# adam-ikari/uvhttp

Measured on AMD Instinct MI355X. Metric: WebSocket payload unmask GiB/s (device-resident), 64 KiB frames, 1/2/4/8 GPU, higher is better.
Workload: dtype u8; 1 GPU; C3: 65536 x 64 KiB masked BINARY frames per GPU (C5 shard shape); mode=inplace, frames_per_gpu=65536, payload_bytes_per_frame=65536, wire_bytes_per_frame=65550, parallelism=shard1 (independent frames, no collective)

## Files before the change

uvhttp_amd/__init__.py:

```python
from __future__ import annotations

import ctypes as C
import os

__all__ = [
    "lib", "LIB_PATH", "FrameHeader", "FrameDesc", "MessageDesc", "BatchSummary", "Batch",
    "WsConnectionStruct", "parse_frame_header", "apply_mask", "WsConnection", "GpuEngine",
    "GpuError", "OPCODES", "FRAME_STATUS", "gen_frame_stride", "GpuPipeline", "Stream",
    "StreamResult", "STREAM_DT", "STREAM_RESULT_DT", "STREAM_RESULT_BYTES", "Batcher",
]

_HERE = os.path.dirname(os.path.abspath(__file__))
LIB_PATH = os.path.join(_HERE, "lib", "libuvhttp_ws_amd.so")
TESTHOOKS_LIB_PATH = os.path.join(_HERE, "lib", "libuvhttp_ws_amd_testhooks.so")

OPCODES = dict(CONTINUATION=0x0, TEXT=0x1, BINARY=0x2, CLOSE=0x8, PING=0x9, PONG=0xA)
FRAME_STATUS = {
    0: "OK", 1: "INCOMPLETE", 2: "SKIPPED", -1: "ERR_PARSE", -2: "ERR_RSV", -3: "ERR_CONTROL",
    -4: "ERR_UNMASKED", -5: "ERR_TOO_BIG", -6: "ERR_BUFFER", -7: "ERR_FRAGMENT",
    -8: "ERR_MESSAGE", -9: "ERR_LAYOUT", -10: "ERR_CAPACITY", -11: "ERR_DEVICE",
}
FLAG_FIN, FLAG_MASK, FLAG_MSG_END = 0x01, 0x02, 0x20


# ... 201 lines not shown
    if _LIB is None:
        _LIB = load_library(LIB_PATH)
    return _LIB


_TESTHOOKS = None


def test_hooks_library() -> C.CDLL:
    global _TESTHOOKS
    if _TESTHOOKS is None:
        _TESTHOOKS = load_library(TESTHOOKS_LIB_PATH)
    return _TESTHOOKS


EXPERIMENT_KNOBS = (
    "UVHTTP_WS_MAX_POLLS", "UVHTTP_WS_SCRATCH_POOL", "UVHTTP_WS_PLAN_FPT", "UVHTTP_WS_EPOCH_START",
    "UVHTTP_WS_BUILD_SMALL", "UVHTTP_WS_FUSED", "UVHTTP_WS_FUSED_MAX", "UVHTTP_WS_PLAN_WIDE",
    "UVHTTP_WS_REC_SCAN", "UVHTTP_WS_BUILD_FRAMES", "UVHTTP_WS_COMPACT", "UVHTTP_WS_WALK_SINGLE",
    "UVHTTP_WS_WALK_FUSE", "UVHTTP_WS_DESC_SCAN", "UVHTTP_WS_WALK_REC",
    "UVHTTP_WS_WALK", "UVHTTP_WS_TIME_CHAIN", "UVHTTP_WS_SPEC", "UVHTTP_WS_SPEC_MAX",
    "UVHTTP_WS_SUMMARY_FAST", "UVHTTP_WS_TILE", "UVHTTP_WS_TIMING_FENCE", "UVHTTP_WS_PIPE_IN_FLIGHT",
    "UVHTTP_TLS_CRYPT_GRID", "UVHTTP_WS_BATCHER_TRACE", "UVHTTP_WS_BATCHER_FAIL_EVERY",
    "UVHTTP_WS_COPY_SSE2", "UVHTTP_WS_DESC_EMIT", "UVHTTP_WS_STREAM_SPEC")


def experiment_knobs_set():
    return [k for k in EXPERIMENT_KNOBS if k in os.environ]


def default_library() -> C.CDLL:
    return test_hooks_library() if experiment_knobs_set() else lib()


def load_library(path: str) -> C.CDLL:
    if not os.path.exists(path):
        raise ImportError(f"{path} missing: run `make` (or __graft_entry__.build())")
    try:
        import torch
    except ImportError:
        pass
    L = C.CDLL(path)
    vp, u32, u64, i32 = C.c_void_p, C.c_uint32, C.c_uint64, C.c_int32
    sig = {
        "uvhttp_ws_amd_version": (C.c_char_p, []),
        "uvhttp_ws_parse_frame_header": (C.c_int, [vp, C.c_size_t, C.POINTER(FrameHeader),
                                                   C.POINTER(C.c_size_t)]),
# ... 881 lines not shown
```

uvhttp_amd/csrc/ws_gpu.hip:

```cpp
#include <hip/hip_runtime.h>

#include <stdint.h>
#include <stdio.h>
#include <stdlib.h>
#include <string.h>

#include <vector>

#include "uvhttp_ws_amd.h"
#include "ws_engine_int.h"

namespace {

constexpr int kBlock = 256;
constexpr uint64_t kMapTile = 16384;
constexpr uint64_t kScatterAvg = 26624;
constexpr uint32_t kMaxFrames = 1u << 26;
constexpr uint32_t kNoFrame = 0xFFFFFFFFu;
constexpr uint32_t kMaxEpoch = (1u << 30) - 1;

typedef uint32_t u32x4 __attribute__((ext_vector_type(4)));

struct ScanElem {
    int32_t last_data;
// ... 157 lines not shown
    ScanElem* group_agg;
    ScanElem* block_incl;
    ScanElem* block_excl;
    LbRec* rec_a;
    LbRec* rec_p;
    uint32_t* counters;
    uint64_t* tile_first;
    uint64_t* first_bad;
    uint64_t* spec_bad;
    uint64_t* arena_first;
    uint32_t* ctl;
    void* recs;
    void* parts;
    uint8_t* info;
};

constexpr int kCtlEpoch = 0;
constexpr int kCtlDone = 1;
constexpr int kCtlFaultEp = 2;
constexpr int kCtlFaults = 3;
constexpr int kCtlGate = 4;
constexpr int kCtlSpecOff = 5;
constexpr int kCtlSpecBreak = 6;
constexpr int kCtlWords = 7;
constexpr uint32_t kMaxHostEpoch = kMaxEpoch / 2;

__device__ inline uint64_t tag_of(uint32_t epoch, uint32_t frame) {
    return ((uint64_t)epoch << 32) | (uint32_t)~frame;
}
__device__ inline void tag_claim(uint64_t* p, uint32_t epoch, uint32_t frame, uint32_t cas) {
    unsigned long long* q = reinterpret_cast<unsigned long long*>(p);
    const unsigned long long mine = tag_of(epoch, frame);
    if (!cas) {
        atomicMax(q, mine);
        return;
    }
    unsigned long long cur = atomicMax(q, mine);
    while ((uint32_t)(cur >> 32) > epoch) {
        const unsigned long long seen = atomicCAS(q, cur, mine);
        if (seen == cur) return;
        cur = seen;
        if ((uint32_t)(cur >> 32) <= epoch) {
            atomicMax(q, mine);
            return;
        }
    }
}
// ... 105 lines not shown
    uint64_t frame_stride;
    double stride_inv;
    FrameRec8* recs;
    uint32_t n;
    int32_t max_frame_size;
    int32_t max_message_size;
    int32_t is_server;
    uint64_t n_tiles;
    uint8_t* arena;
    uint64_t arena_cap;
    uint64_t n_arena_tiles;
    const uvhttp_ws_stream_t* streams;
    const uint32_t* n_dev;
    uvhttp_ws_stream_result_t* s_results;
    const uint32_t* s_over;
    uint32_t n_streams;
    uint32_t epoch;
    uint32_t dev_epoch;
    uint32_t max_polls;
    uvhttp_ws_batch_summary_t* summary;
    uint32_t plan_frames;
    uint64_t* stamp;
    uint64_t spec_P;
    uint32_t gate;
    uint32_t cas_claims;
    uvhttp_ws_message_desc_t* msgs;
};

constexpr uint32_t kStampRing = 128, kStampKinds = 16, kStampBegin = 256, kStampEnd = 4096;
constexpr uint64_t kStampPer = kStampBegin + kStampEnd;
constexpr uint64_t kStampLow = (1ull << 40) - 1;
constexpr uint32_t kStampTagPeriod = (1u << 24) - 1;
constexpr uint64_t kStampWords = (uint64_t)kStampRing * kStampKinds * kStampPer;

__host__ __device__ inline uint32_t stamp_tag(uint32_t epoch) { return epoch % kStampTagPeriod + 1u; }
__device__ inline uint64_t* stamp_slot(uint64_t* st, uint32_t epoch, uint32_t kind) {
    return st + ((uint64_t)(epoch % kStampRing) * kStampKinds + kind) * kStampPer;
}
__host__ __device__ inline bool stamp_sampled(uint64_t g) {
    return g < 1024 || (g < 65536 ? (g & 63) == 63 : (g & 1023) == 1023);
}
__host__ __device__ inline uint32_t stamp_end_word(uint64_t g, uint32_t wave) {
    const uint64_t blk = g < 1024 ? g : g < 65536 ? 1024 + (g >> 6) : 2048 + (g >> 10);
    return (uint32_t)((blk * 4 + (wave & 3)) % kStampEnd);
}
__device__ inline uint64_t stamp_clock() {
// ... 497 lines not shown
template <int FPT>
__device__ inline void plan_pass2(const BatchArgs& a, uvhttp_ws_frame_desc_t* desc,
                                  uvhttp_ws_message_desc_t* msgs, const Workspace& ws, uint32_t i0,
                                  uint32_t n, ScanElem run, uvhttp_ws_frame_desc_t (&dv)[FPT]) {
#pragma unroll
    for (int k = 0; k < FPT; ++k) {
        const uint32_t i = i0 + k;
        if (i < n) {
            const SegInfo g = seg_info(a, i, n);
            ScanElem e = scan_identity();
            if (dv[k].status == UVHTTP_WS_FRAME_OK) e = scan_elem_of(dv[k], (int32_t)i, g.head);
            else if (g.head) e.bits = kHead;
            resolve_one(a, msgs, ws, i, n, g, run, dv[k]);
            store_desc(desc, i, dv[k]);
            run = scan_combine(run, e);
        }
    }
}

template <int FPT, int NT = kBlock, bool REC = false>
__global__ __launch_bounds__(NT) void k_plan(BatchArgs a, uvhttp_ws_frame_desc_t* desc,
                                                 uvhttp_ws_message_desc_t* msgs, Workspace ws) {
    resolve_epoch(a, ws);
    if (a.gate && ws.ctl[kCtlGate] != a.epoch) return;
    StampScope stamp_(a.stamp, a.epoch, UVHTTP_WS_STAMP_PLAN);
    __shared__ uint32_t s_ticket;
    if (threadIdx.x == 0) {
        const uint32_t t =
            __hip_atomic_fetch_add(&ws.counters[0], 1u, __ATOMIC_RELAXED, __HIP_MEMORY_SCOPE_AGENT);
        if (t + 1 == gridDim.x)
            __hip_atomic_store(&ws.counters[0], 0u, __ATOMIC_RELAXED, __HIP_MEMORY_SCOPE_AGENT);
        s_ticket = t;
    }
    __syncthreads();
    const uint32_t b = s_ticket;
    const uint32_t n = nframes(a);
    const uint32_t i0 = (b * NT + threadIdx.x) * FPT;
    if constexpr (REC) {
        ScanElem tagg = scan_identity();
        FrameRec8 r[FPT];
        const uint32_t ilast = n ? n - 1 : 0;
#pragma unroll
        for (int k = 0; k < FPT; ++k) r[k] = a.recs[i0 + k < n ? i0 + k : ilast];
#pragma unroll
        for (int k = 0; k < FPT; ++k) {
            const uint32_t i = i0 + k;
            if (i < n) {
// ... 225 lines not shown
    if (pe <= va || ps >= va + 16) return;
    const uint32_t rk = rotr32(key, 8u * (uint32_t)((va - ps) & 3u));
    if (ps <= va && va + 16 <= pe) {
        m = u32x4{rk, rk, rk, rk};
        return;
    }
    const int lo = ps > va ? (int)(ps - va) : 0;
    const int hi = pe < va + 16 ? (int)(pe - va) : 16;
    m.x |= rk & lane_bytes(lo, hi, 0);
    m.y |= rk & lane_bytes(lo, hi, 1);
    m.z |= rk & lane_bytes(lo, hi, 2);
    m.w |= rk & lane_bytes(lo, hi, 3);
}

__device__ inline bool any_bits(const u32x4& m) { return (m.x | m.y | m.z | m.w) != 0u; }

constexpr int kStoreAux = 18;
__host__ inline void inplace_tile_shape(uint64_t avg, int& blk, int& vpt) {
    if (avg >= 12288) blk = 64, vpt = 1;
    else if (avg >= 2560) blk = 64, vpt = 2;
    else blk = 256, vpt = avg >= 2048 ? 2 : 4;
}

constexpr uint32_t kFastFrames = 8;
template <int BLOCK, int VPT>
__device__ __forceinline__ void unmask_tile(BatchArgs a,
                                            const uvhttp_ws_frame_desc_t* __restrict__ desc,
                                            const Workspace& ws, uint64_t tile_base,
                                            uint32_t& n_out, uint32_t& nb_out, StampScope& ss) {
    constexpr uint64_t kT = (uint64_t)BLOCK * VPT * 16;
    __shared__ uint64_t s_ps[BLOCK];
    __shared__ uint64_t s_pe[BLOCK];
    __shared__ uint32_t s_key[BLOCK];

    const uint64_t t0 = (tile_base + ss.anchor_s(blockIdx.x)) * kT;
    const uint64_t vend = a.wire_len;
    const uint64_t full_end = vend & ~(uint64_t)15;
    const uint64_t clamp_va = full_end ? full_end - 16 : 0;

    u32x4 data[VPT];
    uint64_t va[VPT];
#pragma unroll
    for (int v = 0; v < VPT; ++v) {
        va[v] = t0 + ((uint64_t)v * BLOCK + threadIdx.x) * 16u;
        const uint64_t la = va[v] < full_end ? va[v] : clamp_va;
        data[v] = __builtin_nontemporal_load(reinterpret_cast<const u32x4*>(a.wire + la));
    }

    resolve_epoch(a, ws);
    const uint32_t n = nframes(a);
    const uint32_t nb = first_bad_of(a, ws, n);
    n_out = n;
    nb_out = nb;
    if (nb == 0 || n == 0 || t0 >= vend) return;
    const uint32_t last = (nb < n ? nb : n) - 1;
    const uint64_t c0 = t0 / kMapTile, c1 = (t0 + kT - 1) / kMapTile + 1;
    const uint32_t f0 = tag_get(ws.tile_first[c0], a.epoch, kNoFrame);
    uint32_t f1 = (c1 < a.n_tiles) ? tag_get(ws.tile_first[c1], a.epoch, kNoFrame) : last;
    if (f0 > last) return;
    if (f1 > last || f1 < f0) f1 = last;

    u32x4 m[VPT];
#pragma unroll
    for (int v = 0; v < VPT; ++v) m[v] = u32x4{0, 0, 0, 0};

    if (f1 - f0 < kFastFrames) {
        if (a.streams) {
            for (uint32_t f = f0; f <= f1; ++f) {
                const uint64_t ps = desc[f].payload_off;
                const uint64_t len = desc[f].payload_len;
                const uint32_t key = desc[f].masking_key;
// ... 67 lines not shown
                const uint32_t mw[4] = {m[v].x, m[v].y, m[v].z, m[v].w};
                for (uint64_t bq = 0; full_end + bq < vend; ++bq) {
                    const uint8_t mb = (uint8_t)(mw[bq >> 2] >> (8 * (bq & 3)));
                    if (mb) a.wire[full_end + bq] ^= mb;
                }
            }
        }
    }
}

__device__ inline void device_result(uvhttp_ws_stream_result_t& r);
__device__ inline void capacity_result(uvhttp_ws_stream_result_t& r);
__device__ inline void stream_fix(const BatchArgs& a, const Workspace& ws) {
    const bool fault = ws.ctl[kCtlFaultEp] == a.epoch;
    if (!fault && *a.s_over != a.epoch) return;
    for (uint32_t j = threadIdx.x; j < a.n_streams; j += blockDim.x) {
        uvhttp_ws_stream_result_t o = a.s_results[j];
        if (fault) device_result(o);
        else if (o.n_frames) capacity_result(o);
        a.s_results[j] = o;
    }
}

template <int BLOCK, int VPT>
__global__ __launch_bounds__(BLOCK) void k_unmask_inplace(
    BatchArgs a, const uvhttp_ws_frame_desc_t* __restrict__ desc, Workspace ws,
    uint64_t tile_base) {
    StampScope stamp_(a.stamp, a.epoch, UVHTTP_WS_STAMP_PAYLOAD, false, tile_base);
    uint32_t n, nb;
    unmask_tile<BLOCK, VPT>(a, desc, ws, tile_base, n, nb, stamp_);
    if (!a.streams && tile_base + blockIdx.x < (a.n + BLOCK - 1) / BLOCK) {
        resolve_epoch(a, ws);
        finalize_frames(a, const_cast<uvhttp_ws_frame_desc_t*>(desc), ws,
                        (uint32_t)(tile_base + blockIdx.x), BLOCK, nb);
    }
    if (a.s_results && tile_base + blockIdx.x == 0) {
        resolve_epoch(a, ws);
        stream_fix(a, ws);
    }
}

constexpr uint64_t kFusedMinStride = 64;
constexpr uint64_t kFusedMaxAvg = 2560;

__device__ inline u32x4 lds_window(const u32x4* tile, uint32_t r) {
    const u32x4 v0 = tile[r >> 4], v1 = tile[(r >> 4) + 1];
    uint64_t x0 = v0.x | ((uint64_t)v0.y << 32), x1 = v0.z | ((uint64_t)v0.w << 32);
    uint64_t x2 = v1.x | ((uint64_t)v1.y << 32);
    const uint64_t x3 = v1.z | ((uint64_t)v1.w << 32);
    const uint32_t dd = r & 15;
    if (dd & 8) {
        x0 = x1;
        x1 = x2;
// ... 251 lines not shown
            }
        }
    }
}

__device__ inline void remask_range(uint8_t* wire, uint64_t ps, uint64_t pe, uint32_t key) {
    const int lane = threadIdx.x & 63;
    const uint64_t a0 = (ps + 15) & ~(uint64_t)15, a1 = pe & ~(uint64_t)15;
    if (a0 >= a1) {
        for (uint64_t b = ps + lane; b < pe; b += 64) wire[b] ^= (uint8_t)(key >> (8 * ((b - ps) & 3)));
        return;
    }
    for (uint64_t b = ps + lane; b < a0; b += 64) wire[b] ^= (uint8_t)(key >> (8 * ((b - ps) & 3)));
    for (uint64_t b = a1 + lane; b < pe; b += 64) wire[b] ^= (uint8_t)(key >> (8 * ((b - ps) & 3)));
    const uint32_t rk = rotr32(key, 8u * (uint32_t)((a0 - ps) & 3u));
    for (uint64_t v = a0 + 16ull * lane; v < a1; v += 16ull * 64) {
        u32x4* p = reinterpret_cast<u32x4*>(wire + v);
        *p = *p ^ u32x4{rk, rk, rk, rk};
    }
}

constexpr uint32_t kFixupBlocks = 1024;

__global__ __launch_bounds__(kBlock) void k_fixup(BatchArgs a, uvhttp_ws_frame_desc_t* desc,
                                                  Workspace ws) {
    resolve_epoch(a, ws);
    StampScope stamp_(a.stamp, a.epoch, UVHTTP_WS_STAMP_FIXUP);
    const uint32_t n = a.n;
    const uint32_t nb = first_bad_of(a, ws, n);
    const bool fault = device_fault(a, ws);
    const uint64_t tid = (uint64_t)blockIdx.x * kBlock + threadIdx.x;
    const uint64_t nthreads = (uint64_t)gridDim.x * kBlock;
    if (blockIdx.x == 0 && threadIdx.x < 64) {
        if (fault) {
            if (threadIdx.x == 0) {
                uvhttp_ws_batch_summary_t s;
                memset(&s, 0, sizeof(s));
                s.n_frames = n;
                s.status = -1;
                s.first_status = UVHTTP_WS_FRAME_ERR_DEVICE;
                *a.summary = s;
            }
        } else {
            write_summary(a, desc, ws, nb);
        }
    }
    if (nb >= n) return;
    for (uint64_t i = tid; i < n; i += nthreads)
        if (i > nb || fault) skip_desc(a, desc, i);
    const uint64_t wave = tid >> 6, nwaves = nthreads >> 6;
// ... 874 lines not shown
    }
    __syncthreads();
    *total = all;
    return pre + inc - v;
}


template <int BLOCK, int VPT>
__global__ __launch_bounds__(BLOCK) void k_scatter_compact(
    BatchArgs a, const uvhttp_ws_frame_desc_t* __restrict__ desc, Workspace ws,
    uint64_t arena_bytes_cap, uint64_t tile_base) {
    StampScope stamp_(a.stamp, a.epoch, UVHTTP_WS_STAMP_PAYLOAD, false, tile_base);
    scatter_tile<BLOCK, VPT>(a, desc, ws, arena_bytes_cap, tile_base + stamp_.anchor_s(blockIdx.x));
    if (tile_base + blockIdx.x < (a.n + BLOCK - 1) / BLOCK) {
        resolve_epoch(a, ws);
        finalize_frames(a, const_cast<uvhttp_ws_frame_desc_t*>(desc), ws,
                        (uint32_t)(tile_base + blockIdx.x), BLOCK, first_bad_of(a, ws, a.n));
    }
}

__global__ __launch_bounds__(kBlock) void k_spec_fix(BatchArgs a, uvhttp_ws_frame_desc_t* desc,
                                                     Workspace ws, uint64_t n_tiles) {
    resolve_epoch(a, ws);
    if (a.gate && ws.ctl[kCtlGate] != a.epoch) return;
    StampScope stamp_(a.stamp, a.epoch, UVHTTP_WS_STAMP_FIXUP);
    const uint32_t n = a.n;
    const uint32_t nb = first_bad_of(a, ws, n);
    const bool slow = tag_get(*ws.spec_bad, a.epoch, n) < nb && !device_fault(a, ws);
    if (slow) {
        for (uint64_t t = blockIdx.x; t < n_tiles; t += gridDim.x)
            scatter_tile<kBlock, 4>(a, desc, ws, a.arena_cap, t);
    }
    const uint32_t nblk = (n + kBlock - 1) / kBlock;
    for (uint32_t blk = blockIdx.x; blk < (nblk ? nblk : 1); blk += gridDim.x)
        finalize_frames(a, desc, ws, blk, kBlock, nb, slow);
}
struct WalkArgs {
    const uint8_t* wire;
    uint64_t wire_len;
    const uvhttp_ws_stream_t* streams;
    uint32_t n_streams;
    uint32_t max_frames;
    const uint64_t* read_end;
    uint32_t n_reads_total;
    uint32_t single;
    uint32_t* agg;
    uvhttp_ws_stream_result_t* results;
// ... 2107 lines not shown
            for (int k = 0; k < 4; ++k) w[hs + k] = (uint8_t)(key >> (8 * k));
        }
        const uint64_t b = wi * 8;
        if (b < plen) {
            const uint64_t r = splitmix64(seed + ((uint64_t)i << 32) + wi);
            uint8_t* pl = w + hs + 4;
            for (int k = 0; k < 8 && b + k < plen; ++k)
                pl[b + k] = (uint8_t)(r >> (8 * k)) ^ (uint8_t)(key >> (8 * ((b + k) & 3)));
        }
    }
}

__global__ __launch_bounds__(kBlock) void k_epoch(uint32_t* ctl, uint64_t* ws_words,
                                                  uint64_t n_ws, uint64_t* bs_words,
                                                  uint64_t n_bs) {
    const uint32_t e = *reinterpret_cast<volatile uint32_t*>(ctl + kCtlEpoch);
    const bool wrap = e >= kMaxEpoch || e <= kMaxHostEpoch;
    if (wrap) {
        const uint64_t stride = (uint64_t)gridDim.x * kBlock;
        for (uint64_t k = (uint64_t)blockIdx.x * kBlock + threadIdx.x; k < n_ws; k += stride)
            ws_words[k] = 0;
        for (uint64_t k = (uint64_t)blockIdx.x * kBlock + threadIdx.x; k < n_bs; k += stride)
            bs_words[k] = 0;
    }
    __syncthreads();
    if (threadIdx.x == 0) {
        __threadfence();
        const uint32_t t =
            __hip_atomic_fetch_add(&ctl[kCtlDone], 1u, __ATOMIC_ACQ_REL, __HIP_MEMORY_SCOPE_AGENT);
        if (t + 1 == gridDim.x) {
            __hip_atomic_store(&ctl[kCtlDone], 0u, __ATOMIC_RELAXED, __HIP_MEMORY_SCOPE_AGENT);
            __hip_atomic_store(&ctl[kCtlEpoch], wrap ? kMaxHostEpoch + 1 : e + 1, __ATOMIC_RELEASE,
                               __HIP_MEMORY_SCOPE_AGENT);
        }
    }
}

}

struct uvhttp_ws_gpu_engine {
    int device;
    void* ws_mem;
    size_t ws_bytes;
    uint32_t cap_frames;
    uint64_t cap_tiles, cap_arena_tiles;
    Workspace ws;
    int timing;
    uint64_t timing_calls;
    int tile_block, tile_vpt;
    uint32_t epoch;
    int plan_fpt;
    int fused_off;
    uint64_t fused_max_avg;
    int rec_lookback;
    int plan_wide;
    int walk_mode;
    void* ss_mem;
    uint32_t ss_frames, ss_reads;
    StreamScratch ss;
    void* wt_mem;
    uint64_t wt_cap;
    void* wr_mem;
    uint64_t wr_cap;
    int wr_rec_on;
    int walk_single_off;
    int walk_fuse;
    int desc_scan_off;
    int stream_spec;
    void* sp_mem;
    uint32_t sp_streams;
    uint64_t sp_tiles;
    int spec_on;
    uint64_t spec_max_avg;
    int time_chain;
    void* bs_mem;
    uint64_t bs_tiles;
    int build_small;
    uint64_t build_frames_max;
    int compact_mode;
    int sum_fast;
    uvhttp_ws_frame_desc_t* dscr;
    uint64_t dscr_cap;
    void* u8_mem;
    uint64_t u8_bytes;
    uint32_t* ctl;
    uint32_t faults_seen;
    uint32_t max_polls;
    uint64_t* stamp_mem;
    int stamp_on;
    int capturing;
// ... 37 lines not shown
}

#ifdef UVWS_EXPERIMENTS
static void experiment_knobs(uvhttp_ws_gpu_engine_t* e) {
    if (const char* mp = getenv("UVHTTP_WS_MAX_POLLS")) e->max_polls = (uint32_t)strtoul(mp, nullptr, 0);
    if (const char* po = getenv("UVHTTP_WS_SCRATCH_POOL")) e->pool_ok &= atoi(po) != 0;
    if (const char* fp = getenv("UVHTTP_WS_PLAN_FPT")) e->plan_fpt = atoi(fp);
    if (const char* ep = getenv("UVHTTP_WS_EPOCH_START")) {
        const unsigned long v = strtoul(ep, nullptr, 0);
        e->epoch = v < kMaxHostEpoch ? (uint32_t)v : 0;
    }
    if (const char* bs = getenv("UVHTTP_WS_BUILD_SMALL")) e->build_small = atoi(bs);
    if (const char* fu = getenv("UVHTTP_WS_FUSED")) e->fused_off = atoi(fu) == 0;
    if (const char* fm = getenv("UVHTTP_WS_FUSED_MAX")) e->fused_max_avg = strtoull(fm, nullptr, 10);
    if (const char* pw = getenv("UVHTTP_WS_PLAN_WIDE")) e->plan_wide = atoi(pw) != 0;
    if (const char* rs = getenv("UVHTTP_WS_REC_SCAN")) e->rec_lookback = strcmp(rs, "3pass") != 0;
    if (const char* bf = getenv("UVHTTP_WS_BUILD_FRAMES")) e->build_frames_max = strtoull(bf, nullptr, 10);
    if (const char* cm = getenv("UVHTTP_WS_COMPACT"))
        e->compact_mode = strcmp(cm, "gather") == 0 ? 1 : strcmp(cm, "scatter") == 0 ? 2 : 0;
    if (const char* ws = getenv("UVHTTP_WS_WALK_SINGLE")) e->walk_single_off = atoi(ws) == 0;
    if (const char* wf = getenv("UVHTTP_WS_WALK_FUSE")) e->walk_fuse = atoi(wf) != 0;
    if (const char* ds = getenv("UVHTTP_WS_DESC_SCAN")) e->desc_scan_off = atoi(ds) == 0;
    if (const char* sq = getenv("UVHTTP_WS_STREAM_SPEC")) e->stream_spec = atoi(sq) != 0;
    if (const char* wr = getenv("UVHTTP_WS_WALK_REC")) e->wr_rec_on = atoi(wr) != 0;
    if (const char* wm = getenv("UVHTTP_WS_WALK"))
        e->walk_mode = strcmp(wm, "lane") == 0 ? 1 : strcmp(wm, "wave") == 0 ? 2 : 0;
    if (const char* tc = getenv("UVHTTP_WS_TIME_CHAIN")) e->time_chain = atoi(tc) != 0;
    if (const char* sp2 = getenv("UVHTTP_WS_SPEC")) e->spec_on = atoi(sp2) != 0;
    if (const char* sm = getenv("UVHTTP_WS_SPEC_MAX")) e->spec_max_avg = strtoull(sm, nullptr, 10);
    if (const char* sf = getenv("UVHTTP_WS_SUMMARY_FAST")) e->sum_fast = atoi(sf) != 0;
    if (const char* de = getenv("UVHTTP_WS_DESC_EMIT")) e->desc_emit = atoi(de);
    if (const char* tl = getenv("UVHTTP_WS_TILE")) {
        int tb = 0, tv = 0;
        if (sscanf(tl, "%dx%d", &tb, &tv) == 2) (void)uvhttp_ws_gpu_engine_set_tile(e, tb, tv);
    }
}
#endif

int uvhttp_ws_gpu_engine_create(int device, uvhttp_ws_gpu_engine_t** out) {
    if (!out) return UVHTTP_WS_GPU_EINVAL;
    *out = nullptr;
    int count = 0;
    if (hipGetDeviceCount(&count) != hipSuccess || count <= 0 || device < 0 || device >= count)
        return UVHTTP_WS_GPU_ENODEV;
    hipDeviceProp_t prop;
    if (hipGetDeviceProperties(&prop, device) != hipSuccess) return UVHTTP_WS_GPU_ENODEV;
    if (strncmp(prop.gcnArchName, "gfx950", 6) != 0) return UVHTTP_WS_GPU_ENODEV;
    uvhttp_ws_gpu_engine_t* e = (uvhttp_ws_gpu_engine_t*)calloc(1, sizeof(*e));
    if (!e) return UVHTTP_WS_GPU_ENOMEM;
    e->device = device;
    e->max_polls = kMaxPolls;
    e->fused_max_avg = kFusedMaxAvg;
    e->rec_lookback = 1;
    e->plan_wide = 0;
    e->build_frames_max = 4096;
    e->wr_rec_on = 1;
    e->spec_on = 1;
    e->spec_max_avg = kFusedMaxAvg;
    e->sum_fast = 1;
    e->desc_emit = 2;
    e->stream_spec = 1;
    {
        int prev = 0;
        (void)hipGetDevice(&prev);
        (void)hipSetDevice(device);
        hipError_t h = hipMalloc(&e->ctl, kCtlWords * sizeof(uint32_t));
        if (h == hipSuccess) h = hipMemset(e->ctl, 0, kCtlWords * sizeof(uint32_t));
        if (h == hipSuccess) h = hipDeviceSynchronize();
        (void)hipSetDevice(prev);
        if (h != hipSuccess) {
            if (e->ctl) (void)hipFree(e->ctl);
            free(e);
            return UVHTTP_WS_GPU_ENOMEM;
        }
    }
    {
        int pools = 0;
        if (hipDeviceGetAttribute(&pools, hipDeviceAttributeMemoryPoolsSupported, device) != hipSuccess)
            pools = 0;
        e->pool_ok = pools ? 1 : 0;
    }
#ifdef UVWS_EXPERIMENTS
    experiment_knobs(e);
#endif
// ... 339 lines not shown
        e->ev_created++;
    }
    (void)hipEventRecord(e->ev[2 * k], s);
    return k;
}

static void timing_end(uvhttp_ws_gpu_engine_t* e, int k, hipStream_t s) {
    if (k < 0) return;
    (void)hipEventRecord(e->ev[2 * k + 1], s);
    e->ev_used = k + 1;
}


static uint32_t next_epoch(uvhttp_ws_gpu_engine_t* e, hipStream_t s) {
    if (e->capturing) {
        hipLaunchKernelGGL(k_epoch, dim3(64), dim3(kBlock), 0, s, e->ctl, (uint64_t*)e->ws_mem,
                           (uint64_t)(e->ws_mem ? e->ws_bytes / 8 : 0), (uint64_t*)e->bs_mem,
                           (uint64_t)(e->bs_mem ? e->bs_tiles * sizeof(BuildRec) / 8 : 0));
        return 0;
    }
    if (e->epoch >= kMaxHostEpoch) {
        (void)hipMemsetAsync(e->ws_mem, 0, e->ws_bytes, s);
        if (e->bs_mem) (void)hipMemsetAsync(e->bs_mem, 0, e->bs_tiles * sizeof(BuildRec), s);
        e->epoch = 0;
    }
    return ++e->epoch;
}

struct CallScope {
    uvhttp_ws_gpu_engine_t* e;
    ~CallScope() { e->capturing = 0; }
};

static void call_begin(uvhttp_ws_gpu_engine_t* e, hipStream_t s) {
    hipStreamCaptureStatus cs = hipStreamCaptureStatusNone;
    if (hipStreamIsCapturing(s, &cs) != hipSuccess) cs = hipStreamCaptureStatusNone;
    e->capturing = cs == hipStreamCaptureStatusActive;
    if (e->capturing) e->captured_ever = 1;
    if (!e->capturing && e->have_last && e->last_stream != s) {
        if (!e->order_ev) (void)hipEventCreateWithFlags(&e->order_ev, hipEventDisableTiming);
        if (e->order_ev && hipEventRecord(e->order_ev, e->last_stream) == hipSuccess)
            (void)hipStreamWaitEvent(s, e->order_ev, 0);
    }
    e->last_stream = s;
    e->have_last = 1;
}
// ... 6 lines not shown
    return prev;
}

int uvws_call_leave(uvhttp_ws_gpu_engine_t* e, int prev_device, const char* what) {
    e->capturing = 0;
    const hipError_t h = hipGetLastError();
    if (prev_device != e->device) (void)hipSetDevice(prev_device);
    if (h != hipSuccess) return set_err(e, UVHTTP_WS_GPU_ELAUNCH, what, h);
    return UVHTTP_WS_GPU_OK;
}

int uvws_set_err(uvhttp_ws_gpu_engine_t* e, int code, const char* what) {
    return set_err(e, code, what, hipSuccess);
}

static void launch_plan(uvhttp_ws_gpu_engine_t* e, BatchArgs& a, uint32_t n_cap,
                        uvhttp_ws_frame_desc_t* d_desc, uvhttp_ws_message_desc_t* d_msgs,
                        hipStream_t s) {
    int fpt = e->plan_fpt;
    if (fpt != 1 && fpt != 2 && fpt != 4 && fpt != 8 && fpt != 16) {
        const uint64_t max_blocks = a.recs ? 256 : 512;
        fpt = 1;
        while (fpt < 16 && ((uint64_t)n_cap + kBlock * fpt - 1) / (kBlock * fpt) > max_blocks) fpt *= 2;
    }
    if (a.recs && e->plan_wide) {
        int wf = 1;
        while (wf < 4 && ((uint64_t)n_cap + 1024 * wf - 1) / (1024 * wf) > 256) wf *= 2;
        const uint32_t wper = 1024 * wf;
        a.plan_frames = wper;
        const uint32_t wgrid = n_cap ? (n_cap + wper - 1) / wper : 1;
        if (wf == 1) hipLaunchKernelGGL((k_plan<1, 1024>), dim3(wgrid), dim3(1024), 0, s, a, d_desc, d_msgs, e->ws);
        else if (wf == 2) hipLaunchKernelGGL((k_plan<2, 1024>), dim3(wgrid), dim3(1024), 0, s, a, d_desc, d_msgs, e->ws);
        else hipLaunchKernelGGL((k_plan<4, 1024>), dim3(wgrid), dim3(1024), 0, s, a, d_desc, d_msgs, e->ws);
        return;
    }
    const uint32_t per = kBlock * fpt;
    a.plan_frames = per;
    const uint32_t grid = n_cap ? (n_cap + per - 1) / per : 1;
    if (a.recs) {
        switch (fpt) {
            case 1: hipLaunchKernelGGL((k_plan<1, kBlock, true>), dim3(grid), dim3(kBlock), 0, s, a, d_desc, d_msgs, e->ws); break;
            case 2: hipLaunchKernelGGL((k_plan<2, kBlock, true>), dim3(grid), dim3(kBlock), 0, s, a, d_desc, d_msgs, e->ws); break;
            case 4: hipLaunchKernelGGL((k_plan<4, kBlock, true>), dim3(grid), dim3(kBlock), 0, s, a, d_desc, d_msgs, e->ws); break;
            case 8: hipLaunchKernelGGL((k_plan<8, kBlock, true>), dim3(grid), dim3(kBlock), 0, s, a, d_desc, d_msgs, e->ws); break;
            default: hipLaunchKernelGGL((k_plan<16, kBlock, true>), dim3(grid), dim3(kBlock), 0, s, a, d_desc, d_msgs, e->ws); break;
        }
// ... 195 lines not shown
    if (fb == B && fv == V)                                                                      \
        hipLaunchKernelGGL((k_unmask_stride<B, V>), dim3(grid_p), dim3(B), 0, s, a, e->ws, tb);  \
    else
            UVWS_FUSED(64, 1) UVWS_FUSED(64, 2) UVWS_FUSED(64, 4) UVWS_FUSED(128, 1)
            UVWS_FUSED(128, 2) UVWS_FUSED(256, 1) UVWS_FUSED(256, 2) UVWS_FUSED(256, 4) {
                if (prev != e->device) (void)hipSetDevice(prev);
                return set_err(e, UVHTTP_WS_GPU_EINVAL, "unsupported fused tile shape", hipSuccess);
            }
#undef UVWS_FUSED
        }
        timing_end(e, ftk, s);
        if (e->rec_lookback) {
            launch_plan(e, a, a.n, d_desc, d_msgs, s);
        } else {
            constexpr int kRecFpt = 4;
            a.plan_frames = kBlock * kRecFpt;
            const uint32_t nblk = (a.n + a.plan_frames - 1) / a.plan_frames;
            hipLaunchKernelGGL(k_rec_reduce<kRecFpt>, dim3(nblk), dim3(kBlock), 0, s, a, e->ws);
            hipLaunchKernelGGL(k_rec_scan, dim3(1), dim3(kScanBlock), 0, s, e->ws, nblk);
            hipLaunchKernelGGL(k_rec_resolve<kRecFpt>, dim3(nblk), dim3(kBlock), 0, s, a, d_desc,
                               d_msgs, e->ws);
        }
        const uint32_t fx = (a.n + kBlock - 1) / kBlock;
        hipLaunchKernelGGL(k_fixup, dim3(fx < kFixupBlocks ? fx : kFixupBlocks), dim3(kBlock), 0, s, a, d_desc,
                           e->ws);
        hipError_t hf = hipGetLastError();
        if (prev != e->device) (void)hipSetDevice(prev);
        if (hf != hipSuccess) return set_err(e, UVHTTP_WS_GPU_ELAUNCH, "launch", hf);
        return UVHTTP_WS_GPU_OK;
    }
    const bool no_desc = !d_desc;
    if (!d_desc && !(d_desc = desc_scratch(e, a.n, s))) {
        if (prev != e->device) (void)hipSetDevice(prev);
        return set_err(e, UVHTTP_WS_GPU_ENOMEM, "descriptor scratch (reserve before capturing)", hipSuccess);
    }
    const uint64_t spec_p = spec_payload(b->frame_stride);
    const bool spec = arena && !b->frame_off && e->spec_on && a.n > 0 && spec_p &&
                      b->wire_len / a.n <= e->spec_max_avg && e->compact_mode != 1 &&
                      b->frame_stride >= kFusedMinStride && b->wire_len > 0 &&
                      b->wire_len < (1ull << 52) && arena_cap < (1ull << 52) &&
                      (uint64_t)(a.n - 1) <= (b->wire_len - 1) / b->frame_stride;
    if (spec) {
        a.recs = reinterpret_cast<FrameRec8*>(e->ws.recs);
        a.stride_inv = 1.0 / (double)b->frame_stride;
        a.spec_P = spec_p;
        constexpr uint64_t kSt = 256ull * 4 * 16;
        const uint64_t s_tiles = (b->wire_len + kSt - 1) / kSt;
        const bool sum_c = no_desc && sum_ok(e, b) && arena_cap / spec_p >= a.n;
        const bool desc_c = !no_desc && e->desc_emit && sum_ok(e, b) && arena_cap / spec_p >= a.n;
        if (sum_c) a.recs = reinterpret_cast<FrameRec8*>(e->ws.recs);
        const int stk = timing_begin(e, s);
        for (uint64_t tb = 0; tb < s_tiles; tb += (1ull << 24)) {
            const uint32_t grid_s = (uint32_t)((s_tiles - tb) < (1ull << 24) ? (s_tiles - tb) : (1ull << 24));
            if (desc_c)
                hipLaunchKernelGGL((k_unmask_stride<256, 4, true, kLeaveBoth>), dim3(grid_s), dim3(256), 0,
                                   s, a, e->ws, tb);
            else if (sum_c)
                hipLaunchKernelGGL((k_unmask_stride<256, 4, true, kLeaveInfo>), dim3(grid_s), dim3(256), 0, s, a,
                                   e->ws, tb);
            else
                hipLaunchKernelGGL((k_unmask_stride<256, 4, true>), dim3(grid_s), dim3(256), 0, s, a, e->ws, tb);
        }
        timing_end(e, stk, s);
        if (sum_c) {
            const uint32_t n_parts = (a.n + kBlock * kScanFpt - 1) / (kBlock * kScanFpt);
            hipLaunchKernelGGL(k_sum_scan<true>, dim3(n_parts), dim3(kBlock), 0, s, a, e->ws);
            hipLaunchKernelGGL(k_sum_msgs<>, dim3(n_parts), dim3(kBlock), 0, s, a, e->ws, n_parts, d_msgs,
                               nullptr);
            a.recs = nullptr;
            a.gate = 1;
        } else if (desc_c) {
            const uint32_t n_parts = (a.n + kBlock * kScanFpt - 1) / (kBlock * kScanFpt);
            BatchArgs ai = a;
            ai.recs = reinterpret_cast<FrameRec8*>(e->ws.info);
            hipLaunchKernelGGL((k_sum_scan<true, UVHTTP_WS_STAMP_SUM_SCAN>), dim3(n_parts), dim3(kBlock), 0, s, ai,
                               e->ws);
            hipLaunchKernelGGL(k_sum_msgs<true>, dim3(n_parts), dim3(kBlock), 0, s, a, e->ws, n_parts, d_msgs,
                               d_desc);
            a.gate = 1;
        }
        launch_plan(e, a, a.n, d_desc, d_msgs, s);
        const uint32_t nblk = (a.n + kBlock - 1) / kBlock;
        const uint32_t fix_max = a.gate ? 256u : 1024u;
        hipLaunchKernelGGL(k_spec_fix, dim3(nblk < fix_max ? nblk : fix_max), dim3(kBlock), 0, s, a, d_desc,
                           e->ws, s_tiles);
        const hipError_t hs = hipGetLastError();
        if (prev != e->device) (void)hipSetDevice(prev);
        if (hs != hipSuccess) return set_err(e, UVHTTP_WS_GPU_ELAUNCH, "launch", hs);
        return UVHTTP_WS_GPU_OK;
    }
    launch_plan(e, a, a.n, d_desc, d_msgs, s);
    int blk = e->tile_block, vpt = e->tile_vpt;
    const uint64_t avg = a.n ? b->wire_len / a.n : 0;
    const bool scatter = arena && (e->compact_mode ? e->compact_mode == 2 : avg < kScatterAvg);
    if (!blk) {
        if (!arena) {
            inplace_tile_shape(avg, blk, vpt);
        } else if (scatter) {
            blk = avg >= 32768 ? 64 : 256;
            vpt = avg >= 32768 ? 1 : avg >= 2048 ? 2 : 4;
            if (avg >= 2048 && avg < 16384) vpt = 4;
        } else {
// ... 789 lines not shown
```

Before: 3158 GiB/s.

## Add stride-speculative in-place unmask path that skips planning for uniform frames

Adds a speculative in-place path for fixed-stride batches. It computes frame boundaries arithmetically from the stride, checks each frame header against a precomputed header image, and unmasks payload tiles directly, so the plan kernel does not have to run first. The first tile of each frame writes a record or descriptor, and any non-uniform frame sets a break flag in the control words. The plan and fixup kernels are gated on that flag and only do full work when speculation fails; otherwise fixup writes a synthetic summary. This removes the serial planning cost before unmasking, at the price of extra header checks per tile and added complexity in the fallback.

```diff
diff --git a/uvhttp_amd/__init__.py b/uvhttp_amd/__init__.py
--- a/uvhttp_amd/__init__.py
+++ b/uvhttp_amd/__init__.py
@@ -247,7 +247,7 @@
     "UVHTTP_WS_WALK", "UVHTTP_WS_TIME_CHAIN", "UVHTTP_WS_SPEC", "UVHTTP_WS_SPEC_MAX",
     "UVHTTP_WS_SUMMARY_FAST", "UVHTTP_WS_TILE", "UVHTTP_WS_TIMING_FENCE", "UVHTTP_WS_PIPE_IN_FLIGHT",
     "UVHTTP_TLS_CRYPT_GRID", "UVHTTP_WS_BATCHER_TRACE", "UVHTTP_WS_BATCHER_FAIL_EVERY",
-    "UVHTTP_WS_COPY_SSE2", "UVHTTP_WS_DESC_EMIT", "UVHTTP_WS_STREAM_SPEC")
+    "UVHTTP_WS_COPY_SSE2", "UVHTTP_WS_DESC_EMIT", "UVHTTP_WS_STREAM_SPEC", "UVHTTP_WS_STRIDE_SPEC")
 
 
 def experiment_knobs_set():
diff --git a/uvhttp_amd/csrc/ws_gpu.hip b/uvhttp_amd/csrc/ws_gpu.hip
--- a/uvhttp_amd/csrc/ws_gpu.hip
+++ b/uvhttp_amd/csrc/ws_gpu.hip
@@ -203,7 +203,8 @@
 constexpr int kCtlGate = 4;
 constexpr int kCtlSpecOff = 5;
 constexpr int kCtlSpecBreak = 6;
-constexpr int kCtlWords = 7;
+constexpr int kCtlStrideBreak = 7;
+constexpr int kCtlWords = 8;
 constexpr uint32_t kMaxHostEpoch = kMaxEpoch / 2;
 
 __device__ inline uint64_t tag_of(uint32_t epoch, uint32_t frame) {
@@ -355,6 +356,8 @@
     uint32_t plan_frames;
     uint64_t* stamp;
     uint64_t spec_P;
+    uint64_t spec_hx, spec_hm;
+    uint32_t spec_hx2, spec_hm2;
     uint32_t gate;
     uint32_t cas_claims;
     uvhttp_ws_message_desc_t* msgs;
@@ -898,7 +901,7 @@
 __global__ __launch_bounds__(NT) void k_plan(BatchArgs a, uvhttp_ws_frame_desc_t* desc,
                                                  uvhttp_ws_message_desc_t* msgs, Workspace ws) {
     resolve_epoch(a, ws);
-    if (a.gate && ws.ctl[kCtlGate] != a.epoch) return;
+    if (a.gate && ws.ctl[a.gate] != a.epoch) return;
     StampScope stamp_(a.stamp, a.epoch, UVHTTP_WS_STAMP_PLAN);
     __shared__ uint32_t s_ticket;
     if (threadIdx.x == 0) {
@@ -1170,8 +1173,42 @@
     else blk = 256, vpt = avg >= 2048 ? 2 : 4;
 }
 
+__device__ __forceinline__ bool sspec_image(const BatchArgs& a, const u32x4& hv) {
+    const uint64_t hlo = (uint64_t)hv.x | ((uint64_t)hv.y << 32);
+    return ((hlo ^ a.spec_hx) & a.spec_hm) == 0 &&
+           ((hv.z ^ a.spec_hx2) & a.spec_hm2) == 0 && (hv.x & 3u) != 3u;
+}
+__device__ __forceinline__ uint32_t sspec_key(uint32_t D, const u32x4& hv) {
+    return D == 6 ? (hv.x >> 16) | (hv.y << 16) : D == 8 ? hv.y : (hv.z >> 16) | (hv.w << 16);
+}
+__device__ __forceinline__ void sspec_fill(const BatchArgs& a, uint64_t o, const u32x4& hv,
+                                           uvhttp_ws_frame_desc_t& d) {
+    const uint64_t S = a.frame_stride, P = a.spec_P;
+    d.payload_off = o + (S - P);
+    d.payload_len = P;
+    d.masking_key = sspec_key((uint32_t)(S - P), hv);
+    d.message = 0;
+    d.opcode = (uint8_t)(hv.x & 0xFu);
+    d.flags = (uint8_t)(((hv.x >> 7) & 1u) | UVHTTP_WS_FLAG_MASK);
+    d.header_size = (uint8_t)((uint32_t)(S - P) - 4u);
+    d.status = UVHTTP_WS_FRAME_OK;
+    d.wire_len = (uint32_t)S;
+}
+__device__ __forceinline__ u32x4 load16_dw(const uint8_t* base, uint64_t len, uint64_t o, bool inside) {
+    if (inside) {
+        const uint32_t* p = reinterpret_cast<const uint32_t*>(base + (o & ~(uint64_t)3));
+        const uint32_t w0 = p[0], w1 = p[1], w2 = p[2], w3 = p[3], w4 = p[4];
+        const uint32_t sh = (uint32_t)(o & 3) * 8;
+        auto fun = [sh](uint32_t x, uint32_t y) { return (uint32_t)((((uint64_t)y << 32) | x) >> sh); };
+        return u32x4{fun(w0, w1), fun(w1, w2), fun(w2, w3), fun(w3, w4)};
+    }
+    return load16_at(base, len, o);
+}
+__device__ inline int32_t rel_clamp(uint64_t x, uint64_t t0, uint64_t kT, bool keep_phase);
+__device__ inline void add_mask_rel(u32x4& m, int32_t r, int32_t ps, int32_t pe, uint32_t key);
+
 constexpr uint32_t kFastFrames = 8;
-template <int BLOCK, int VPT>
+template <int BLOCK, int VPT, bool SSPEC = false>
 __device__ __forceinline__ void unmask_tile(BatchArgs a,
                                             const uvhttp_ws_frame_desc_t* __restrict__ desc,
                                             const Workspace& ws, uint64_t tile_base,
@@ -1181,7 +1218,8 @@
     __shared__ uint64_t s_pe[BLOCK];
     __shared__ uint32_t s_key[BLOCK];
 
-    const uint64_t t0 = (tile_base + ss.anchor_s(blockIdx.x)) * kT;
+    const uint64_t tile = tile_base + ss.anchor_s(blockIdx.x);
+    const uint64_t t0 = tile * kT;
     const uint64_t vend = a.wire_len;
     const uint64_t full_end = vend & ~(uint64_t)15;
     const uint64_t clamp_va = full_end ? full_end - 16 : 0;
@@ -1195,6 +1233,120 @@
         data[v] = __builtin_nontemporal_load(reinterpret_cast<const u32x4*>(a.wire + la));
     }
 
+    if constexpr (SSPEC) {
+        const uint32_t n = a.n;
+        n_out = nb_out = n;
+        const uint64_t S = a.frame_stride;
+        const uint32_t S32 = (uint32_t)S, D32 = S32 - (uint32_t)a.spec_P;
+        const uint64_t room = vend - t0;
+        const uint32_t room32 = (room >> 31) ? 0x7FFFFFFFu : (uint32_t)room;
+        const uint32_t nrec = room32 < (uint32_t)kT ? room32 : (uint32_t)kT;
+        uint32_t q = (uint32_t)((double)(uint32_t)tile * a.stride_inv);
+        int32_t r = (int32_t)((uint32_t)t0 - q * S32);
+        if (r < 0) {
+            --q;
+            r += (int32_t)S32;
+        } else if (r >= (int32_t)S32) {
+            ++q;
+            r -= (int32_t)S32;
+        }
+        const bool in_slot = q < n;
+        const uint32_t f0 = in_slot ? q : n - 1;
+        const uint64_t o0 = in_slot ? t0 - (uint32_t)r : (uint64_t)f0 * S;
+        const uint32_t r0 = (uint32_t)r;
+        const bool more = f0 + 1 < n;
+        const bool two = more && S32 - r0 < nrec;
+        const u32x4 hv0 = load16_dw(a.wire, vend, o0, in_slot && room32 + r0 >= 20u);
+        u32x4 hv1 = u32x4{0, 0, 0, 0};
+        if (two) hv1 = load16_dw(a.wire, vend, o0 + S, room32 + r0 >= S32 + 20u);
+        const bool fast0 = in_slot && sspec_image(a, hv0) && (more || S32 - r0 <= room32);
+        uvhttp_ws_frame_desc_t od = {};
+        int32_t ps0, pe0;
+        uint32_t key0;
+        if (fast0) {
+            ps0 = (int32_t)D32 - (int32_t)r0;
+            pe0 = (int32_t)S32 - (int32_t)r0;
+            key0 = sspec_key(D32, hv0);
+        } else {
+            (void)parse_hdr(a, f0, seg_info(a, f0, n), o0, hv0, od);
+            ps0 = rel_clamp(od.payload_off, t0, kT, true);
+            pe0 = rel_clamp(od.payload_off + (od.status == UVHTTP_WS_FRAME_OK ? od.payload_len : 0), t0, kT, false);
+            key0 = od.masking_key;
+        }
+        __amdgpu_buffer_rsrc_t rs =
+            __builtin_amdgcn_make_buffer_rsrc(a.wire + t0, 0, (int)nrec, 0x00020000);
+        if (!two && ps0 <= 0 && pe0 >= (int32_t)kT) {
+            const uint32_t rk = rotr32(key0, 8u * ((uint32_t)(-ps0) & 3u));
+#pragma unroll
+            for (int v = 0; v < VPT; ++v) {
+                const u32x4 x = data[v] ^ u32x4{rk, rk, rk, rk};
+                __builtin_amdgcn_raw_buffer_store_b128(
+                    __builtin_bit_cast(__attribute__((ext_vector_type(4))) unsigned int, x), rs,
+                    (uint32_t)((v * BLOCK + threadIdx.x) * 16), 0, kStoreAux);
+            }
+            return;
+        }
+        u32x4 m[VPT];
+#pragma unroll
+        for (int v = 0; v < VPT; ++v) {
+            m[v] = u32x4{0, 0, 0, 0};
+            add_mask_rel(m[v], (int32_t)((v * BLOCK + threadIdx.x) * 16), ps0, pe0, key0);
+        }
+        uint32_t of = o0 >= t0 ? f0 : kNoFrame;
+        bool ofast = fast0;
+        if (two) {
+            const uint64_t o1 = o0 + S;
+            of = f0 + 1;
+            ofast = sspec_image(a, hv1) && (f0 + 2 < n || 2 * S32 - r0 <= room32);
+            int32_t ps1 = (int32_t)(S32 - r0) + (int32_t)D32, pe1 = (int32_t)kT + 64;
+            uint32_t key1 = sspec_key(D32, hv1);
+            if (!ofast) {
+                (void)parse_hdr(a, of, seg_info(a, of, n), o1, hv1, od);
+                ps1 = rel_clamp(od.payload_off, t0, kT, true);
+                pe1 = rel_clamp(od.payload_off + (od.status == UVHTTP_WS_FRAME_OK ? od.payload_len : 0), t0, kT, false);
+                key1 = od.masking_key;
+            }
+#pragma unroll
+            for (int v = 0; v < VPT; ++v)
+                add_mask_rel(m[v], (int32_t)((v * BLOCK + threadIdx.x) * 16), ps1, pe1, key1);
+        }
+#pragma unroll
+        for (int v = 0; v < VPT; ++v) {
+            if (any_bits(m[v]) && va[v] + 16 <= vend) {
+                const u32x4 x = data[v] ^ m[v];
+                __builtin_amdgcn_raw_buffer_store_b128(
+                    __builtin_bit_cast(__attribute__((ext_vector_type(4))) unsigned int, x), rs,
+                    (uint32_t)(va[v] - t0), 0, kStoreAux);
+            }
+        }
+        if (full_end != vend && full_end >= t0 && full_end < t0 + kT) {
+#pragma unroll
+            for (int v = 0; v < VPT; ++v) {
+                if (va[v] == full_end && any_bits(m[v])) {
+                    const uint32_t mw[4] = {m[v].x, m[v].y, m[v].z, m[v].w};
+                    for (uint64_t bq = 0; full_end + bq < vend; ++bq) {
+                        const uint8_t mb = (uint8_t)(mw[bq >> 2] >> (8 * (bq & 3)));
+                        if (mb) a.wire[full_end + bq] ^= mb;
+                    }
+                }
+            }
+        }
+        if (of == kNoFrame || threadIdx.x != 0) return;
+        if (ofast) sspec_fill(a, (uint64_t)of * S, two ? hv1 : hv0, od);
+        a.recs[of] = rec8_of_desc(od);
+        const bool uniform = od.status == UVHTTP_WS_FRAME_OK && (od.opcode == 1 || od.opcode == 2) &&
+                             od.flags == (UVHTTP_WS_FLAG_FIN | UVHTTP_WS_FLAG_MASK) &&
+                             od.payload_len == a.spec_P && od.header_size + 4u == S - a.spec_P;
+        if (!uniform) {
+            resolve_epoch(a, ws);
+            ws.ctl[kCtlStrideBreak] = a.epoch;
+        } else if (desc) {
+            od.message = of;
+            od.flags |= UVHTTP_WS_FLAG_MSG_END;
+            store_desc(const_cast<uvhttp_ws_frame_desc_t*>(desc), of, od);
+        }
+        return;
+    }
     resolve_epoch(a, ws);
     const uint32_t n = nframes(a);
     const uint32_t nb = first_bad_of(a, ws, n);
@@ -1308,13 +1460,14 @@
     }
 }
 
-template <int BLOCK, int VPT>
+template <int BLOCK, int VPT, bool SSPEC = false>
 __global__ __launch_bounds__(BLOCK) void k_unmask_inplace(
     BatchArgs a, const uvhttp_ws_frame_desc_t* __restrict__ desc, Workspace ws,
     uint64_t tile_base) {
     StampScope stamp_(a.stamp, a.epoch, UVHTTP_WS_STAMP_PAYLOAD, false, tile_base);
     uint32_t n, nb;
-    unmask_tile<BLOCK, VPT>(a, desc, ws, tile_base, n, nb, stamp_);
+    unmask_tile<BLOCK, VPT, SSPEC>(a, desc, ws, tile_base, n, nb, stamp_);
+    if constexpr (SSPEC) return;
     if (!a.streams && tile_base + blockIdx.x < (a.n + BLOCK - 1) / BLOCK) {
         resolve_epoch(a, ws);
         finalize_frames(a, const_cast<uvhttp_ws_frame_desc_t*>(desc), ws,
@@ -1612,10 +1765,26 @@
 
 constexpr uint32_t kFixupBlocks = 1024;
 
+template <bool SSPEC = false>
 __global__ __launch_bounds__(kBlock) void k_fixup(BatchArgs a, uvhttp_ws_frame_desc_t* desc,
                                                   Workspace ws) {
     resolve_epoch(a, ws);
     StampScope stamp_(a.stamp, a.epoch, UVHTTP_WS_STAMP_FIXUP);
+    if constexpr (SSPEC) {
+        if (ws.ctl[kCtlStrideBreak] != a.epoch) {
+            if (blockIdx.x == 0 && threadIdx.x == 0) {
+                uvhttp_ws_batch_summary_t s;
+                memset(&s, 0, sizeof(s));
+                s.n_frames = a.n;
+                s.n_delivered = a.n;
+                s.consumed_bytes = (uint64_t)a.n * a.frame_stride;
+                s.payload_bytes = (uint64_t)a.n * a.spec_P;
+                s.n_messages = a.n;
+                *a.summary = s;
+            }
+            return;
+        }
+    }
     const uint32_t n = a.n;
     const uint32_t nb = first_bad_of(a, ws, n);
     const bool fault = device_fault(a, ws);
@@ -2536,7 +2705,7 @@
 __global__ __launch_bounds__(kBlock) void k_spec_fix(BatchArgs a, uvhttp_ws_frame_desc_t* desc,
                                                      Workspace ws, uint64_t n_tiles) {
     resolve_epoch(a, ws);
-    if (a.gate && ws.ctl[kCtlGate] != a.epoch) return;
+    if (a.gate && ws.ctl[a.gate] != a.epoch) return;
     StampScope stamp_(a.stamp, a.epoch, UVHTTP_WS_STAMP_FIXUP);
     const uint32_t n = a.n;
     const uint32_t nb = first_bad_of(a, ws, n);
@@ -4690,6 +4859,7 @@
             ws_words[k] = 0;
         for (uint64_t k = (uint64_t)blockIdx.x * kBlock + threadIdx.x; k < n_bs; k += stride)
             bs_words[k] = 0;
+        if (blockIdx.x == 0 && threadIdx.x == 0) ctl[kCtlStrideBreak] = 0;
     }
     __syncthreads();
     if (threadIdx.x == 0) {
@@ -4734,6 +4904,7 @@
     int walk_single_off;
     int walk_fuse;
     int desc_scan_off;
+    int stride_spec;
     int stream_spec;
     void* sp_mem;
     uint32_t sp_streams;
@@ -4817,6 +4988,7 @@
     if (const char* wf = getenv("UVHTTP_WS_WALK_FUSE")) e->walk_fuse = atoi(wf) != 0;
     if (const char* ds = getenv("UVHTTP_WS_DESC_SCAN")) e->desc_scan_off = atoi(ds) == 0;
     if (const char* sq = getenv("UVHTTP_WS_STREAM_SPEC")) e->stream_spec = atoi(sq) != 0;
+    if (const char* sd = getenv("UVHTTP_WS_STRIDE_SPEC")) e->stride_spec = atoi(sd) != 0;
     if (const char* wr = getenv("UVHTTP_WS_WALK_REC")) e->wr_rec_on = atoi(wr) != 0;
     if (const char* wm = getenv("UVHTTP_WS_WALK"))
         e->walk_mode = strcmp(wm, "lane") == 0 ? 1 : strcmp(wm, "wave") == 0 ? 2 : 0;
@@ -4855,6 +5027,7 @@
     e->sum_fast = 1;
     e->desc_emit = 2;
     e->stream_spec = 1;
+    e->stride_spec = 1;
     {
         int prev = 0;
         (void)hipGetDevice(&prev);
@@ -5240,6 +5413,7 @@
     if (e->epoch >= kMaxHostEpoch) {
         (void)hipMemsetAsync(e->ws_mem, 0, e->ws_bytes, s);
         if (e->bs_mem) (void)hipMemsetAsync(e->bs_mem, 0, e->bs_tiles * sizeof(BuildRec), s);
+        (void)hipMemsetAsync(e->ctl + kCtlStrideBreak, 0, sizeof(uint32_t), s);
         e->epoch = 0;
     }
     return ++e->epoch;
@@ -5292,6 +5466,7 @@
         const uint64_t max_blocks = a.recs ? 256 : 512;
         fpt = 1;
         while (fpt < 16 && ((uint64_t)n_cap + kBlock * fpt - 1) / (kBlock * fpt) > max_blocks) fpt *= 2;
+        if (a.gate == kCtlStrideBreak) fpt = 16;
     }
     if (a.recs && e->plan_wide) {
         int wf = 1;
@@ -5533,7 +5708,7 @@
                                d_msgs, e->ws);
         }
         const uint32_t fx = (a.n + kBlock - 1) / kBlock;
-        hipLaunchKernelGGL(k_fixup, dim3(fx < kFixupBlocks ? fx : kFixupBlocks), dim3(kBlock), 0, s, a, d_desc,
+        hipLaunchKernelGGL(k_fixup<>, dim3(fx < kFixupBlocks ? fx : kFixupBlocks), dim3(kBlock), 0, s, a, d_desc,
                            e->ws);
         hipError_t hf = hipGetLastError();
         if (prev != e->device) (void)hipSetDevice(prev);
@@ -5546,6 +5721,62 @@
         return set_err(e, UVHTTP_WS_GPU_ENOMEM, "descriptor scratch (reserve before capturing)", hipSuccess);
     }
     const uint64_t spec_p = spec_payload(b->frame_stride);
+    int sb = e->tile_block, sv = e->tile_vpt;
+    if (!sb && a.n) inplace_tile_shape(b->wire_len / a.n, sb, sv);
+    const uint64_t mm_lim = (uint64_t)(int64_t)b->max_message_size;
+    const uint64_t mf_lim = (uint64_t)(int64_t)b->max_frame_size;
+    const bool sspec = e->stride_spec && !arena && !b->frame_off && a.n > 0 && b->wire_len > 0 &&
+                       b->wire_len / a.n > e->fused_max_avg && sb == 64 && sv == 2 &&
+                       b->frame_stride >= (uint64_t)sb * sv * 16 && b->frame_stride < (1ull << 30) &&
+                       spec_p != 0 &&
+                       b->wire_len < (1ull << 40) &&
+                       (uint64_t)(a.n - 1) <= (b->wire_len - 1) / b->frame_stride &&
+                       (mm_lim == 0 || mm_lim >= spec_p) && spec_p <= mf_lim &&
+                       b->frame_stride <= (mf_lim > 65536u ? mf_lim : 65536u);
+    if (sspec) {
+        a.recs = reinterpret_cast<FrameRec8*>(e->ws.recs);
+        a.stride_inv = 1.0 / (double)b->frame_stride;
+        BatchArgs ap = a;
+        ap.spec_P = spec_p;
+        {
+            const uint64_t hsz = b->frame_stride - spec_p - 4;
+            uint8_t img[10] = {0, 0, 0, 0, 0, 0, 0, 0, 0, 0}, msk[10] = {0x7C, 0xFF, 0, 0, 0, 0, 0, 0, 0, 0};
+            img[1] = (uint8_t)(0x80 | (hsz == 2 ? spec_p : hsz == 4 ? 126 : 127));
+            for (uint64_t k = 2; k < hsz; ++k) {
+                img[k] = (uint8_t)(spec_p >> (8 * (hsz - 1 - k)));
+                msk[k] = 0xFF;
+            }
+            for (int k = 0; k < 8; ++k) {
+                ap.spec_hx |= (uint64_t)img[k] << (8 * k);
+                ap.spec_hm |= (uint64_t)msk[k] << (8 * k);
+            }
+            ap.spec_hx2 = (uint32_t)img[8] | ((uint32_t)img[9] << 8);
+            ap.spec_hm2 = (uint32_t)msk[8] | ((uint32_t)msk[9] << 8);
+        }
+        const uint64_t s_tile = (uint64_t)sb * sv * 16;
+        BatchArgs ay = ap;
+        ay.stride_inv = (double)s_tile / (double)b->frame_stride;
+        const uint64_t s_tiles = (b->wire_len + s_tile - 1) / s_tile;
+        const uint64_t s_max = (1ull << 24);
+        uvhttp_ws_frame_desc_t* p_desc = no_desc ? nullptr : d_desc;
+        const int stk = timing_begin(e, s);
+        for (uint64_t tb = 0; tb < s_tiles; tb += s_max) {
+            const uint32_t grid_p = (uint32_t)((s_tiles - tb) < s_max ? (s_tiles - tb) : s_max);
+            hipLaunchKernelGGL((k_unmask_inplace<64, 2, true>), dim3(grid_p), dim3(64), 0, s, ay, p_desc,
+                               e->ws, tb);
+        }
+        timing_end(e, stk, s);
+        a.gate = kCtlStrideBreak;
+        launch_plan(e, a, a.n, d_desc, d_msgs, s);
+        ap.plan_frames = a.plan_frames;
+        const uint32_t fx = (a.n + kBlock - 1) / kBlock;
+        hipLaunchKernelGGL(k_fixup<true>, dim3(fx < kFixupBlocks ? fx : kFixupBlocks), dim3(kBlock), 0, s, ap,
+                           d_desc, e->ws);
+        const hipError_t hs = hipGetLastError();
+        if (prev != e->device) (void)hipSetDevice(prev);
+        if (hs != hipSuccess) return set_err(e, UVHTTP_WS_GPU_ELAUNCH, "launch", hs);
+        return UVHTTP_WS_GPU_OK;
+    }
     const bool spec = arena && !b->frame_off && e->spec_on && a.n > 0 && spec_p &&
                       b->wire_len / a.n <= e->spec_max_avg && e->compact_mode != 1 &&
                       b->frame_stride >= kFusedMinStride && b->wire_len > 0 &&
@@ -5579,7 +5810,7 @@
             hipLaunchKernelGGL(k_sum_msgs<>, dim3(n_parts), dim3(kBlock), 0, s, a, e->ws, n_parts, d_msgs,
                                nullptr);
             a.recs = nullptr;
-            a.gate = 1;
+            a.gate = kCtlGate;
         } else if (desc_c) {
             const uint32_t n_parts = (a.n + kBlock * kScanFpt - 1) / (kBlock * kScanFpt);
             BatchArgs ai = a;
@@ -5588,7 +5819,7 @@
                                e->ws);
             hipLaunchKernelGGL(k_sum_msgs<true>, dim3(n_parts), dim3(kBlock), 0, s, a, e->ws, n_parts, d_msgs,
                                d_desc);
-            a.gate = 1;
+            a.gate = kCtlGate;
         }
         launch_plan(e, a, a.n, d_desc, d_msgs, s);
         const uint32_t nblk = (a.n + kBlock - 1) / kBlock;
```

Result: no change. 3156 GiB/s (-0.1%).
